# ssilverman16/particle_col_image_segmentation

Measured on AMD Instinct MI355X. Metric: Mpixels/sec segmented (5-ch 1024x1024 TIFF), ROI mask IoU=1.0, higher is better.
Workload: dtype f32 planes / u8 class maps / int32 labels / f64 ROI sums; 1 GPU; BASELINE config 2: batch of 64 frames 1024x1024x5 float32 per GPU, full kernel chain, inputs resident in HBM; frames_per_gpu=64, height=1024, width=1024, planes=5, parallelism=frames x1, launch=one hipGraph replay per step, 4 in flight, tie_fallback_frames_last_step=0, reference_nan_frames_rank0=0

## Files before the change

particle_col_image_segmentation_amd/csrc/watershed.hip:

```cpp
#include <algorithm>
#include <atomic>
#include <climits>
#include <mutex>
#include <type_traits>

#include "common.h"
#include "tile_rounds.h"

namespace pcseg {

constexpr int WS_T = 64;
constexpr unsigned WS_INF = 0xFFFFFFFFu;
constexpr int WS_CNT0 = 32, WS_CNT_STRIDE = 32, WS_CHANGED_INTS = WS_CNT0 + 16 * WS_CNT_STRIDE;

__device__ __forceinline__ unsigned ws_key(float f)
{
    if (f == 0.0f) f = 0.0f;
    unsigned u = __float_as_uint(f);
    u = (u & 0x80000000u) ? ~u : (u | 0x80000000u);
    return u == WS_INF ? WS_INF - 1 : u;
}

__global__ void __launch_bounds__(256) ws_init_kernel(const float *__restrict__ img, int64_t frame_stride,
                                                       const int *__restrict__ markers, const uint8_t *__restrict__ mask,
                                                       unsigned *__restrict__ val, unsigned *__restrict__ L,
                                                       int *__restrict__ out, int64_t n, int64_t total)
{
    int64_t i = (int64_t)blockIdx.x * blockDim.x + threadIdx.x;
    if (i >= total) return;
    bool m = mask[i] != 0;
    unsigned v = m ? ws_key(img[(i / n) * frame_stride + (i % n)]) : WS_INF;
    int mk = m ? markers[i] : 0;
    val[i] = v;
    L[i] = mk != 0 ? v : WS_INF;
    out[i] = mk;
}

constexpr int WS_LIST_SPAN = 8;
template <typename Body>
__device__ __forceinline__ void ws_for_frames(const int *frame_list, int grid_index, int grid_size, Body &&body)
{
    if (!frame_list) body(grid_index);
    else walk_list(frame_list, frame_list - 1, grid_index, grid_size, body);
}
static inline int ws_frame_span(const int *frame_list, int B) { return frame_list ? (B < WS_LIST_SPAN ? B : WS_LIST_SPAN) : B; }

constexpr int WS_TILE_GRID = 512;

template <typename Body>
__device__ __forceinline__ void ws_for_tile_pixels(int tx, int ty, int H, int W, Body &&body)
{
    const int c = tx * WS_T + (threadIdx.x & 63);
    for (int rr = threadIdx.x >> 6; rr < WS_T; rr += 4) {
        const int r = ty * WS_T + rr;
        if (r < H && c < W) body(r, c);
    }
}

struct RelaxGeom {
    static_assert(WS_T == 64, "relaxation tiles are 64 pixels wide: one wave per sweep quadrant");
    static constexpr int S = WS_T + 2;
    static constexpr int P = WS_T + 4;
    static constexpr int PAD = 8;
    static constexpr int N = S * P + 2 * PAD;
    static constexpr int THREADS = 4 * 64;
    static constexpr int HE = WS_T / 2;
    static constexpr size_t LDS_BYTES = sizeof(uint2) * N;
};

template <int DR, int DC, int P>
__device__ __forceinline__ bool ws_quadrant_sweep(uint2 *sLV, int lane)
{
    unsigned *sLw = reinterpret_cast<unsigned *>(sLV);
    typedef unsigned u2v __attribute__((ext_vector_type(2)));
    unsigned long long diff = 0;
    {
        constexpr int fr = DR > 0 ? 1 : WS_T, hr = DR > 0 ? 0 : WS_T + 1;
        const uint2 c = sLV[fr * P + 1 + lane];
        const unsigned h = sLV[hr * P + 1 + lane].x;
        const unsigned nw = min(c.x, max(c.y, h));
        atomicMin(&sLw[2 * (fr * P + 1 + lane)], nw);
        diff |= __ballot(nw != c.x);
    }
    const int lr = DR > 0 ? lane + 1 : WS_T - lane;
    const uint2 *row = sLV + lr * P;
    const unsigned halo = row[DC > 0 ? 0 : WS_T + 1].x;
    const int u0 = (0 - lane) & 63;
    unsigned left = row[DC > 0 ? u0 : WS_T + 1 - u0].x;
    const int un = (0 - (lane + 1)) & 63;
    unsigned prev = row[DC > 0 ? 1 + un : WS_T - un].x;
    const unsigned a0 = (unsigned)(uintptr_t)(row + (DC > 0 ? 1 : WS_T));
#pragma unroll 1
    for (int j0 = 0; j0 < WS_T; j0 += 8) {
        const int ub = (u0 + j0) & 63;
        const unsigned base_a = DC > 0 ? a0 + 8u * (unsigned)ub : a0 - 8u * (unsigned)ub - 56u;
        const unsigned base_b = DC > 0 ? base_a - 512u : base_a + 512u;
        unsigned ba[8];
        u2v t[8];
#define PCSEG_DS_READ(k)                                                                                                   \
        {                                                                                                                      \
            const unsigned long long wrapped = (((1ull << (k)) - 1ull) << 1) << j0;                \
            asm("v_cndmask_b32_e64 %0, %1, %2, %3" : "=v"(ba[k]) : "v"(base_a), "v"(base_b), "s"(wrapped));                     \
            asm volatile("ds_read_b64 %0, %1 offset:%2" : "=v"(t[k]) : "v"(ba[k]), "n"(DC > 0 ? 8 * (k) : 8 * (7 - (k))));     \
        }
        PCSEG_DS_READ(0) PCSEG_DS_READ(1) PCSEG_DS_READ(2) PCSEG_DS_READ(3)
        PCSEG_DS_READ(4) PCSEG_DS_READ(5) PCSEG_DS_READ(6) PCSEG_DS_READ(7)
#undef PCSEG_DS_READ
        asm volatile("s_waitcnt lgkmcnt(0)" : "+v"(t[0]), "+v"(t[1]), "+v"(t[2]), "+v"(t[3]), "+v"(t[4]), "+v"(t[5]), "+v"(t[6]), "+v"(t[7]));
        unsigned wr[8];
        unsigned long long batch_diff = 0;
#pragma unroll
        for (int k = 0; k < 8; ++k) {
            const unsigned up = (unsigned)__builtin_amdgcn_update_dpp((int)WS_INF, (int)prev, 0x138, 0xF, 0xF, false);
            const unsigned long long at0 = (1ull << k) << j0;
            unsigned lf;
            asm("v_cndmask_b32_e64 %0, %1, %2, %3" : "=v"(lf) : "v"(left), "v"(halo), "s"(at0));
            const unsigned cur = t[k].x, v = t[k].y;
            const unsigned m = min(up, lf);
            const unsigned cand = min(max(v, m), max(min(v, m), cur));
            wr[k] = cand;
            batch_diff |= __ballot(cur != cand);
            left = cand;
            prev = cand;
        }
        if (batch_diff != 0) {
#define PCSEG_DS_MIN(k)                                                                                                             \
            asm volatile("ds_min_u32 %0, %1 offset:%2" : : "v"(ba[k]), "v"(wr[k]), "n"(DC > 0 ? 8 * (k) : 8 * (7 - (k))) : "memory");
            PCSEG_DS_MIN(0) PCSEG_DS_MIN(1) PCSEG_DS_MIN(2) PCSEG_DS_MIN(3)
            PCSEG_DS_MIN(4) PCSEG_DS_MIN(5) PCSEG_DS_MIN(6) PCSEG_DS_MIN(7)
#undef PCSEG_DS_MIN
            diff |= batch_diff;
        }
    }
    return diff != 0;
}

struct WsInputs {
    const float *img;
    int64_t frame_stride;
    const int *markers;
    const uint8_t *mask;
    int *out;
    bool vec;
};


__device__ __forceinline__ void ws_relax_tile(uint2 *sLV, const WsInputs &in, const bool FIRST, unsigned *__restrict__ val,
                                              unsigned *__restrict__ L, uint8_t *__restrict__ dirty_in,
                                              uint8_t *__restrict__ dirty_out, int *__restrict__ any_changed, int H, int W,
                                              const Tiling &cur, const Tiling &nxt, int max_iter, int tx, int ty, int b,
                                              int *__restrict__ list_out = nullptr, int *__restrict__ count_out = nullptr)
{
    using G = RelaxGeom;
    constexpr int T = WS_T, S = G::S, P = G::P, NT = G::THREADS, QW = T / 4;
    const int tid = threadIdx.x;
    if (!FIRST && !take_mark(dirty_in + ((int64_t)b * cur.ny + ty) * cur.nx + tx)) return;
    if (tid == 0) atomicAdd(any_changed + WS_CNT0 + WS_CNT_STRIDE * ((tx + 5 * ty + 3 * b) & 15), 1);
    const int r0 = ty * T - cur.off, c0 = tx * T - cur.off;
    const int64_t fbase = (int64_t)b * H * W;
    auto initial = [&](int r, int c) -> uint2 {
        const int64_t g = fbase + rowoff(r, W) + c;
        if (!in.mask[g]) return make_uint2(WS_INF, WS_INF);
        const unsigned v = ws_key(in.img[(int64_t)b * in.frame_stride + rowoff(r, W) + c]);
        return make_uint2(in.markers[g] != 0 ? v : WS_INF, v);
    };
    if (in.vec) {
        constexpr int QUADS = S * QW, TRIPS = (QUADS + NT - 1) / NT;
        const float *img_f = in.img + (int64_t)b * in.frame_stride;
        const bool halo_thread = tid < 2 * S;
        const int h_lr = tid >> 1, h_lc = (tid & 1) ? S - 1 : 0;
        const int h_r = r0 + h_lr - 1, h_c = c0 + h_lc - 1;
        const bool h_in = halo_thread && h_r >= 0 && h_r < H && h_c >= 0 && h_c < W;
        const int64_t h_p = rowoff(min(max(h_r, 0), H - 1), W) + min(max(h_c, 0), W - 1);
        if (FIRST) {
            float4 f4[TRIPS];
            int4 m4[TRIPS];
            unsigned k4[TRIPS];
#pragma unroll
            for (int t = 0; t < TRIPS; ++t) {
                const int idx = min(tid + NT * t, QUADS - 1);
                const int lr = idx / QW, q = idx % QW;
                const int64_t p = rowoff(min(max(r0 + lr - 1, 0), H - 1), W) + min(max(c0 + 4 * q, 0), W - 4);
                f4[t] = *reinterpret_cast<const float4 *>(img_f + p);
                m4[t] = *reinterpret_cast<const int4 *>(in.markers + fbase + p);
                k4[t] = *reinterpret_cast<const unsigned *>(in.mask + fbase + p);
            }
            const float hf = img_f[h_p];
            const int hm = in.markers[fbase + h_p];
            const uint8_t hk = in.mask[fbase + h_p];
#pragma unroll
            for (int t = 0; t < TRIPS; ++t) {
                const int idx = tid + NT * t;
                if (idx < QUADS) {
                    const int lr = idx / QW, q = idx % QW;
                    const int r = r0 + lr - 1, c = c0 + 4 * q;
                    const bool inside = r >= 0 && r < H && c >= 0 && c < W;
                    const float fv[4] = {f4[t].x, f4[t].y, f4[t].z, f4[t].w};
                    const int mv[4] = {m4[t].x, m4[t].y, m4[t].z, m4[t].w};
                    unsigned key[4];
                    int lab[4];
#pragma unroll
                    for (int j = 0; j < 4; ++j) {
                        const bool msk = inside && ((k4[t] >> (8 * j)) & 255u) != 0;
                        key[j] = msk ? ws_key(fv[j]) : WS_INF;
                        lab[j] = msk ? mv[j] : 0;
                        sLV[lr * P + 1 + 4 * q + j] = make_uint2(lab[j] != 0 ? key[j] : WS_INF, key[j]);
                    }
                    if (inside && lr >= 1 && lr <= T) {
                        const int64_t g = fbase + rowoff(r, W) + c;
                        *reinterpret_cast<uint4 *>(val + g) = make_uint4(key[0], key[1], key[2], key[3]);
                        *reinterpret_cast<int4 *>(in.out + g) = make_int4(lab[0], lab[1], lab[2], lab[3]);
                    }
                }
            }
            if (halo_thread) {
                const bool msk = h_in && hk != 0;
                const unsigned key = msk ? ws_key(hf) : WS_INF;
                sLV[h_lr * P + h_lc] = make_uint2(msk && hm != 0 ? key : WS_INF, key);
            }
        } else {
            uint4 l4[TRIPS], v4[TRIPS];
#pragma unroll
            for (int t = 0; t < TRIPS; ++t) {
                const int idx = min(tid + NT * t, QUADS - 1);
                const int lr = idx / QW, q = idx % QW;
                const int64_t p = fbase + rowoff(min(max(r0 + lr - 1, 0), H - 1), W) + min(max(c0 + 4 * q, 0), W - 4);
                l4[t] = *reinterpret_cast<const uint4 *>(L + p);
                v4[t] = *reinterpret_cast<const uint4 *>(val + p);
            }
            const unsigned hl = L[fbase + h_p], hv = val[fbase + h_p];
#pragma unroll
            for (int t = 0; t < TRIPS; ++t) {
                const int idx = tid + NT * t;
                if (idx < QUADS) {
                    const int lr = idx / QW, q = idx % QW;
                    const int r = r0 + lr - 1, c = c0 + 4 * q;
                    const bool inside = r >= 0 && r < H && c >= 0 && c < W;
                    uint2 *dst = sLV + lr * P + 1 + 4 * q;
                    dst[0] = inside ? make_uint2(l4[t].x, v4[t].x) : make_uint2(WS_INF, WS_INF);
                    dst[1] = inside ? make_uint2(l4[t].y, v4[t].y) : make_uint2(WS_INF, WS_INF);
                    dst[2] = inside ? make_uint2(l4[t].z, v4[t].z) : make_uint2(WS_INF, WS_INF);
                    dst[3] = inside ? make_uint2(l4[t].w, v4[t].w) : make_uint2(WS_INF, WS_INF);
                }
            }
            if (halo_thread) sLV[h_lr * P + h_lc] = h_in ? make_uint2(hl, hv) : make_uint2(WS_INF, WS_INF);
        }
    } else
    for (int i = tid; i < S * S; i += NT) {
        int lr = i / S, lc = i % S;
        int r = r0 + lr - 1, c = c0 + lc - 1;
        uint2 lv = make_uint2(WS_INF, WS_INF);
        if (r >= 0 && r < H && c >= 0 && c < W) {
            if (FIRST) {
                lv = initial(r, c);
                if (lr >= 1 && lr <= T && lc >= 1 && lc <= T) {
                    const int64_t g = fbase + rowoff(r, W) + c;
                    val[g] = lv.y;
                    in.out[g] = lv.y != WS_INF ? in.markers[g] : 0;
                }
            } else {
                lv.x = L[fbase + rowoff(r, W) + c];
                lv.y = val[fbase + rowoff(r, W) + c];
            }
        }
        sLV[lr * P + lc] = lv;
    }
    __syncthreads();
    const bool rim_thread = tid < 8 * G::HE;
    const int e = tid / G::HE, ej = tid % G::HE;
    const int qy = e < 4 ? (e >> 1) : (e & 1), qx = e < 4 ? (e & 1) : ((e >> 1) & 1);
    const int rim_lr = e < 4 ? (qy ? T : 1) : qy * G::HE + ej + 1;
    const int rim_lc = e < 4 ? qx * G::HE + ej + 1 : (qx ? T : 1);
    const unsigned rim_before = rim_thread ? sLV[rim_lr * P + rim_lc].x : 0u;
    const int dir = (tid >> 6) & 3, lane = tid & 63;
    bool changed_any = false;
    bool capped = true;
    for (int iter = 0; iter < max_iter; ++iter) {
        bool changed;
        if (dir == 0) changed = ws_quadrant_sweep<1, 1, P>(sLV, lane);
        else if (dir == 1) changed = ws_quadrant_sweep<1, -1, P>(sLV, lane);
        else if (dir == 2) changed = ws_quadrant_sweep<-1, 1, P>(sLV, lane);
        else changed = ws_quadrant_sweep<-1, -1, P>(sLV, lane);
        if (!__syncthreads_or(changed)) { capped = false; break; }
        changed_any = true;
    }
    if (!FIRST && !changed_any) return;
    if (changed_any) {
        const int r = r0 + rim_lr - 1, c = c0 + rim_lc - 1;
        bool ch = rim_thread && capped;
        if (rim_thread && !capped && r >= 0 && r < H && c >= 0 && c < W) ch = sLV[rim_lr * P + rim_lc].x != rim_before;
        const unsigned long long mine = ((1ull << G::HE) - 1ull) << ((tid & 63) / G::HE * G::HE);
        const unsigned long long edge_changed = __ballot(ch) & mine;
        if (rim_thread && edge_changed && ej == 0) {
            const int oy = (r0 + qy * G::HE + nxt.off) / T, ox = (c0 + qx * G::HE + nxt.off) / T;
            if (oy >= 0 && oy < nxt.ny && ox >= 0 && ox < nxt.nx)
                mark_tile(dirty_out, list_out, count_out, ((int64_t)b * nxt.ny + oy) * nxt.nx + ox);
        }
    }
    __syncthreads();
    if (in.vec) {
#pragma unroll
        for (int t = 0; t < T * QW / NT; ++t) {
            const int idx = tid + NT * t, lr = idx / QW, q = idx % QW;
            const int r = r0 + lr, c = c0 + 4 * q;
            const uint2 *src = sLV + (lr + 1) * P + 1 + 4 * q;
            if (r >= 0 && r < H && c >= 0 && c < W)
                *reinterpret_cast<uint4 *>(L + fbase + rowoff(r, W) + c) = make_uint4(src[0].x, src[1].x, src[2].x, src[3].x);
        }
        return;
    }
    for (int i = tid; i < T * T; i += NT) {
        int lr = i / T, lc = i % T;
        int r = r0 + lr, c = c0 + lc;
        if (r >= 0 && r < H && c >= 0 && c < W) L[fbase + rowoff(r, W) + c] = sLV[(lr + 1) * P + lc + 1].x;
    }
}

__global__ void __launch_bounds__(RelaxGeom::THREADS) ws_relax_kernel(WsInputs in, const bool FIRST, unsigned *__restrict__ val,
                                                                         unsigned *__restrict__ L, uint8_t *__restrict__ dirty_in,
                                                                         uint8_t *__restrict__ dirty_out, int *__restrict__ any_changed,
                                                                         int H, int W, Tiling cur, Tiling nxt, int max_iter,
                                                                         int *__restrict__ list_out, int *__restrict__ count_out)
{
    extern __shared__ __attribute__((aligned(16))) uint2 relax_lds[];
    const TileIndex t = xcd_tile_index();
    ws_relax_tile(relax_lds + RelaxGeom::PAD, in, FIRST, val, L, dirty_in, dirty_out, any_changed, H, W, cur, nxt, max_iter, t.x, t.y,
                     t.z, list_out, count_out);
}

constexpr int WS_LIST_FROM = 4, WS_LIST_GRID = 1024;

__global__ void __launch_bounds__(RelaxGeom::THREADS) ws_relax_list_kernel(WsInputs in, unsigned *__restrict__ val, unsigned *__restrict__ L,
                                                                           uint8_t *__restrict__ dirty_in, uint8_t *__restrict__ dirty_out,
                                                                           int *__restrict__ any_changed, int H, int W, Tiling cur,
                                                                           Tiling nxt, int max_iter, TileList tiles,
                                                                           int *__restrict__ list_out, int *__restrict__ count_out)
{
    extern __shared__ __attribute__((aligned(16))) uint2 relax_lds[];
    for_tiles(tiles, [&](const int b, const int tx, const int ty) {
        ws_relax_tile(relax_lds + RelaxGeom::PAD, in, false, val, L, dirty_in, dirty_out, any_changed, H, W, cur, nxt, max_iter, tx, ty, b,
                      list_out, count_out);
        __syncthreads();
    });
}

__global__ void __launch_bounds__(RelaxGeom::THREADS) ws_relax_tail_kernel(WsInputs in, unsigned *__restrict__ val, unsigned *__restrict__ L,
                                                                           uint8_t *__restrict__ dirtyA, uint8_t *__restrict__ dirtyB,
                                                                           int *__restrict__ any_changed, int *__restrict__ not_converged,
                                                                           int *__restrict__ exact_flags, int H, int W, Tiling t0,
                                                                           Tiling t1, int first_round, int max_rounds)
{
    extern __shared__ __attribute__((aligned(16))) uint2 relax_lds[];
    const int b = blockIdx.x;
    const int rounds = tail_rounds<RelaxGeom::THREADS>(
        b, dirtyA, dirtyB, first_round, max_rounds, t0, t1, [](const int) { return true; },
        [&](const Tiling &cur, const Tiling &nxt, const int tx, const int ty, uint8_t *din, uint8_t *dout) {
            ws_relax_tile(relax_lds + RelaxGeom::PAD, in, false, val, L, din, dout, any_changed, H, W, cur, nxt, 100000, tx, ty, b);
        });
    if (rounds < 0 && threadIdx.x == 0) { *not_converged = 1; exact_flags[b] = 1; }
}

__device__ __forceinline__ bool ws_active(const uint8_t *active, int b, int r, int c, int tilesX, int tilesY)
{
    return active == nullptr || active[((int64_t)b * tilesY + r / WS_T) * tilesX + c / WS_T] != 0;
}

__global__ void __launch_bounds__(256) ws_list_tiles_kernel(const int *__restrict__ frame_list, const uint8_t *__restrict__ active, int ntpf,
                                                             int *__restrict__ tile_list)
{
    ws_for_frames(frame_list, blockIdx.x, gridDim.x, [&](const int b) {
        for (int t = threadIdx.x; t < ntpf; t += 256)
            if (active[(int64_t)b * ntpf + t]) tile_list[atomicAdd(&tile_list[-1], 1)] = b * ntpf + t;
    });
}

constexpr int UF_TW = 64, UF_TH = 32, UF_SW = UF_TW + 2, UF_SH = UF_TH + 2;
constexpr int UF_LNS = UF_TW * UF_TH;
constexpr int UF_NS = 1 << 30;

__device__ __forceinline__ int vfind_lds(int *par, int v)
{
    int p;
    while ((p = ld_lds(par + (v & (UF_LNS - 1)))) != v) {
        const int g = ld_lds(par + (p & (UF_LNS - 1)));
        if (g != p) st_lds(par + (v & (UF_LNS - 1)), g);
        v = g;
    }
    return v;
}
__device__ __forceinline__ void vunite_lds(int *par, int a, int b)
{
    for (;;) {
        a = vfind_lds(par, a);
        b = vfind_lds(par, b);
        if (a == b) return;
        if (a < b) { int t = a; a = b; b = t; }
        int old = atomicMin(&par[a & (UF_LNS - 1)], b);
        if (old == a) return;
        a = old;
    }
}
__device__ __forceinline__ bool vwalk_ok(int x, int p, int n) { return (unsigned)p <= (unsigned)x && (p & (UF_NS - 1)) < n; }

__device__ __forceinline__ void vunite_glb(int *par, int p, int q, int n, int *corrupt)
{
    int a = ld_agent(par + p), b = ld_agent(par + q);
    bool ok = a >= 0 && b >= 0 && (a & (UF_NS - 1)) < n && (b & (UF_NS - 1)) < n;
    while (ok) {
        for (;;) {
            if (a == b) return;
            const int pa = ld_agent(par + (a & (UF_NS - 1))), pb = ld_agent(par + (b & (UF_NS - 1)));
            if (pa == a && pb == b) break;
            if (!vwalk_ok(a, pa, n) || !vwalk_ok(b, pb, n)) { ok = false; break; }
            const int ga = ld_agent(par + (pa & (UF_NS - 1))), gb = ld_agent(par + (pb & (UF_NS - 1)));
            if (!vwalk_ok(pa, ga, n) || !vwalk_ok(pb, gb, n)) { ok = false; break; }
            if (pa != a) {
                if (ga != pa) __hip_atomic_store(par + (a & (UF_NS - 1)), ga, __ATOMIC_RELAXED, __HIP_MEMORY_SCOPE_AGENT);
                a = ga;
            }
            if (pb != b) {
                if (gb != pb) __hip_atomic_store(par + (b & (UF_NS - 1)), gb, __ATOMIC_RELAXED, __HIP_MEMORY_SCOPE_AGENT);
                b = gb;
            }
        }
        if (!ok) break;
        if (a == b) return;
        if (a < b) { int t = a; a = b; b = t; }
        int old = atomicMin(par + (a & (UF_NS - 1)), b);
        if (old == a) return;
        if (!vwalk_ok(a, old, n)) break;
        a = old;
    }
    walk_corrupt(corrupt);
}
__device__ __forceinline__ int vwalk_root(const int *par, int x, int n, bool &bad)
{
    int q;
    while ((q = par[x & (UF_NS - 1)]) != x) {
        if (!vwalk_ok(x, q, n)) {
            bad = true;
            break;
        }
        x = q;
    }
    return x;
}

template <typename KeyT>
__device__ __forceinline__ void ws_uf_tile_frame(KeyT *sK, int *par, uint8_t *sM, const int b, const int tile_x, const int tile_y,
                                                 const KeyT *__restrict__ K,
                                                 const int *__restrict__ F, const uint8_t *__restrict__ active,
                                                 int *__restrict__ parent, uint8_t *__restrict__ minmask, uint8_t *__restrict__ bad,
                                                 int H, int W, int tilesX, int tilesY)
{
    const KeyT KINF = ~(KeyT)0;
    const int r0 = tile_y * UF_TH, c0 = tile_x * UF_TW;
    if (!ws_active(active, b, r0, c0, tilesX, tilesY)) return;
    const int64_t fbase = (int64_t)b * H * W;
    if (sizeof(KeyT) == 4 && (W & 3) == 0 && c0 + UF_TW <= W && (((uintptr_t)K) & 15) == 0) {
        constexpr int QUADS = UF_SH * (UF_TW / 4), TRIPS = (QUADS + 255) / 256;
        uint4 kq[TRIPS];
#pragma unroll
        for (int t = 0; t < TRIPS; ++t) {
            const int i = min((int)threadIdx.x + 256 * t, QUADS - 1);
            const int r = r0 + i / (UF_TW / 4) - 1;
            kq[t] = *reinterpret_cast<const uint4 *>(K + fbase + rowoff(min(max(r, 0), H - 1), W) + c0 + 4 * (i % (UF_TW / 4)));
        }
        const int hl = min((int)threadIdx.x, UF_SH * 2 - 1);
        const int hr = r0 + (hl >> 1) - 1, hx = (hl & 1) ? UF_TW : -1, hc = c0 + hx;
        const KeyT hv = K[fbase + rowoff(min(max(hr, 0), H - 1), W) + min(max(hc, 0), W - 1)];
#pragma unroll
        for (int t = 0; t < TRIPS; ++t) {
            const int i = (int)threadIdx.x + 256 * t;
            if (i < QUADS) {
                const int lr = i / (UF_TW / 4), r = r0 + lr - 1;
                const bool in = r >= 0 && r < H;
                KeyT *dst = sK + lr * UF_SW + 1 + 4 * (i % (UF_TW / 4));
                dst[0] = in ? (KeyT)kq[t].x : KINF; dst[1] = in ? (KeyT)kq[t].y : KINF;
                dst[2] = in ? (KeyT)kq[t].z : KINF; dst[3] = in ? (KeyT)kq[t].w : KINF;
            }
        }
        if (threadIdx.x < UF_SH * 2) sK[(hl >> 1) * UF_SW + hx + 1] = (hr >= 0 && hr < H && hc >= 0 && hc < W) ? hv : KINF;
    } else {
        constexpr int TRIPS = (UF_SH * UF_SW + 255) / 256;
        KeyT kv[TRIPS];
#pragma unroll
        for (int t = 0; t < TRIPS; ++t) {
            const int i = min((int)threadIdx.x + 256 * t, UF_SH * UF_SW - 1);
            const int r = r0 + i / UF_SW - 1, c = c0 + i % UF_SW - 1;
            kv[t] = K[fbase + rowoff(min(max(r, 0), H - 1), W) + min(max(c, 0), W - 1)];
        }
#pragma unroll
        for (int t = 0; t < TRIPS; ++t) {
            const int i = (int)threadIdx.x + 256 * t;
            const int r = r0 + i / UF_SW - 1, c = c0 + i % UF_SW - 1;
            if (i < UF_SH * UF_SW) sK[i] = (r >= 0 && r < H && c >= 0 && c < W) ? kv[t] : KINF;
        }
    }
    __syncthreads();
    int self[UF_LNS / 256];
    int fv[UF_LNS / 256];
#pragma unroll
    for (int k = 0; k < UF_LNS / 256; ++k) {
        const int t = threadIdx.x + k * 256;
        fv[k] = F[fbase + rowoff(min(r0 + t / UF_TW, H - 1), W) + min(c0 + t % UF_TW, W - 1)];
    }
#pragma unroll
    for (int k = 0; k < UF_LNS / 256; ++k) {
        const int t = threadIdx.x + k * 256;
        const int lr = t / UF_TW, lc = t % UF_TW;
        const int r = r0 + lr, c = c0 + lc;
        const int i = (lr + 1) * UF_SW + lc + 1;
        int v = -1;
        if ((unsigned)(sK[i] >> (8 * sizeof(KeyT) - 32)) != WS_INF)
            v = fv[k] != 0 ? t : t + UF_LNS;
        uint8_t m8 = 0;
        if (v >= UF_LNS) {
            const KeyT ku = sK[i - UF_SW], kl = sK[i - 1], kr = sK[i + 1], kd = sK[i + UF_SW];
            const KeyT m = min(min(ku, kd), min(kl, kr));
            if (m != KINF) m8 = (ku == m ? 1 : 0) | (kl == m ? 2 : 0) | (kr == m ? 4 : 0) | (kd == m ? 8 : 0);
        }
        self[k] = v;
        sM[t] = m8;
        if (r < H && c < W) {
            minmask[fbase + rowoff(r, W) + c] = m8;
            if (fv[k] != 0) bad[fbase + rowoff(r, W) + c] = 0;
        }
    }
    __syncthreads();
#pragma unroll
    for (int k = 0; k < UF_LNS / 256; ++k) {
        const int t = threadIdx.x + k * 256;
        const int lc = t % UF_TW;
        const bool joins_left = lc > 0 && ((sM[t] & 2) || (sM[t - 1] & 4));
        const unsigned long long heads = __ballot(!joins_left);
        const unsigned long long seeds = __ballot(self[k] >= 0 && self[k] < UF_LNS);
        const unsigned long long upto = heads & (lc == 63 ? ~0ull : ((2ull << lc) - 1ull));
        const int start = 63 - __clzll((long long)upto);
        const unsigned long long later = lc == 63 ? 0ull : (heads >> (lc + 1));
        const int end = later ? lc + (__ffsll((long long)later) - 1) : 63;
        const unsigned long long run = (end == 63 ? ~0ull : ((2ull << end) - 1ull)) & ~((1ull << start) - 1ull);
        const unsigned long long run_seeds = seeds & run;
        int root = -1;
        if (self[k] >= 0) {
            if (run_seeds) root = (t - lc) + (__ffsll((long long)run_seeds) - 1);
            else root = (t - lc) + start + UF_LNS;
        }
        par[t] = root;
    }
    __syncthreads();
#pragma unroll
    for (int k = 0; k < UF_LNS / 256; ++k) {
        const int t = threadIdx.x + k * 256;
        const int lr = t / UF_TW, lc = t % UF_TW;
        if (lr == 0 || self[k] < 0) continue;
        const uint8_t m = sM[t], mu = sM[t - UF_TW];
        if (!((m & 1) || (mu & 8))) continue;
        if (lc > 0) {
            const uint8_t ml = sM[t - 1], mul = sM[t - UF_TW - 1];
            const bool same_run = (m & 2) || (ml & 4), same_run_up = (mu & 2) || (mul & 4), left_vertical = (ml & 1) || (mul & 8);
            if (same_run && same_run_up && left_vertical) continue;
        }
        vunite_lds(par, par[t], par[t - UF_TW]);
    }
    __syncthreads();
    for (int t = threadIdx.x; t < UF_TH * UF_TW; t += 256) {
        const int r = r0 + t / UF_TW, c = c0 + t % UF_TW;
        if (r >= H || c >= W) continue;
        int v = -1;
        if (par[t] >= 0) {
            const int root = vfind_lds(par, par[t]);
            const int lt = root & (UF_LNS - 1);
            v = ((r0 + lt / UF_TW) * W + c0 + lt % UF_TW) | (root >= UF_LNS ? UF_NS : 0);
        }
        parent[fbase + rowoff(r, W) + c] = v;
    }
}

template <typename KeyT, bool LIST>
__global__ void __launch_bounds__(256) ws_uf_tile_kernel(TileList tiles, const KeyT *__restrict__ K, const int *__restrict__ F,
                                                          const uint8_t *__restrict__ active, int *__restrict__ parent,
                                                          uint8_t *__restrict__ minmask, uint8_t *__restrict__ bad, int H, int W,
                                                          int tilesX, int tilesY)
{
    __shared__ KeyT sK[UF_SH * UF_SW];
    __shared__ int par[UF_TH * UF_TW];
    __shared__ uint8_t sM[UF_LNS];
// ... 1135 lines not shown
```

Before: 16780 Mpixels/s.

## Track changed rows in relaxation sweeps and confirm convergence early via row checks

Each quadrant sweep now returns a bitmask of the rows it changed instead of a single flag. On non-first visits, when only a few rows (dilated by one) changed, each wave checks those rows for any remaining fixed-point violations, and the tile stops iterating early if none are found. This is meant to save the extra full confirming sweep per tile visit. The cost is an extra barrier and the row-check work, plus the risk of stopping before true convergence if the check misses a case.

After: 17020 Mpixels/s (median of 5 runs). 1.5% higher.

```diff
diff --git a/particle_col_image_segmentation_amd/csrc/watershed.hip b/particle_col_image_segmentation_amd/csrc/watershed.hip
--- a/particle_col_image_segmentation_amd/csrc/watershed.hip
+++ b/particle_col_image_segmentation_amd/csrc/watershed.hip
@@ -69,18 +69,19 @@
 };
 
 template <int DR, int DC, int P>
-__device__ __forceinline__ bool ws_quadrant_sweep(uint2 *sLV, int lane)
+__device__ __forceinline__ unsigned long long ws_quadrant_sweep(uint2 *sLV, int lane)
 {
     unsigned *sLw = reinterpret_cast<unsigned *>(sLV);
     typedef unsigned u2v __attribute__((ext_vector_type(2)));
     unsigned long long diff = 0;
+    constexpr int fr = DR > 0 ? 1 : WS_T, hr = DR > 0 ? 0 : WS_T + 1;
+    unsigned long long first_row_diff;
     {
-        constexpr int fr = DR > 0 ? 1 : WS_T, hr = DR > 0 ? 0 : WS_T + 1;
         const uint2 c = sLV[fr * P + 1 + lane];
         const unsigned h = sLV[hr * P + 1 + lane].x;
         const unsigned nw = min(c.x, max(c.y, h));
         atomicMin(&sLw[2 * (fr * P + 1 + lane)], nw);
-        diff |= __ballot(nw != c.x);
+        first_row_diff = __ballot(nw != c.x);
     }
     const int lr = DR > 0 ? lane + 1 : WS_T - lane;
     const uint2 *row = sLV + lr * P;
@@ -132,7 +133,9 @@
             diff |= batch_diff;
         }
     }
-    return diff != 0;
+    unsigned long long rows = DR > 0 ? diff : __brevll(diff);
+    if (first_row_diff != 0) rows |= 1ull << (fr - 1);
+    return rows;
 }
 
 struct WsInputs {
@@ -144,6 +147,36 @@
     bool vec;
 };
 
+
+constexpr int WS_CONFIRM_ROWS = 16;
+
+template <int P>
+__device__ __forceinline__ bool ws_rows_violated(const uint2 *sLV, unsigned long long rows, int wave, int lane)
+{
+    unsigned long long mine = rows & (0x1111111111111111ull << __builtin_amdgcn_readfirstlane(wave));
+    const int first = __ffsll(mine);
+    bool violated = false;
+    while (mine != 0) {
+        int r[4];
+#pragma unroll
+        for (int j = 0; j < 4; ++j) {
+            const int b = __ffsll(mine);
+            mine &= mine - 1;
+            r[j] = b != 0 ? b : first;
+        }
+        uint2 c[4];
+        unsigned m[4];
+#pragma unroll
+        for (int j = 0; j < 4; ++j) {
+            const uint2 *p = sLV + r[j] * P + 1 + lane;
+            c[j] = p[0];
+            m[j] = min(min(p[-P].x, p[P].x), min(p[-1].x, p[1].x));
+        }
+#pragma unroll
+        for (int j = 0; j < 4; ++j) violated |= c[j].x > max(c[j].y, m[j]);
+    }
+    return violated;
+}
 
 __device__ __forceinline__ void ws_relax_tile(uint2 *sLV, const WsInputs &in, const bool FIRST, unsigned *__restrict__ val,
                                               unsigned *__restrict__ L, uint8_t *__restrict__ dirty_in,
@@ -275,14 +308,32 @@
     const int dir = (tid >> 6) & 3, lane = tid & 63;
     bool changed_any = false;
     bool capped = true;
+    __shared__ unsigned long long changed_rows[2][4];
+    __shared__ int row_verdict[4];
     for (int iter = 0; iter < max_iter; ++iter) {
-        bool changed;
-        if (dir == 0) changed = ws_quadrant_sweep<1, 1, P>(sLV, lane);
-        else if (dir == 1) changed = ws_quadrant_sweep<1, -1, P>(sLV, lane);
-        else if (dir == 2) changed = ws_quadrant_sweep<-1, 1, P>(sLV, lane);
-        else changed = ws_quadrant_sweep<-1, -1, P>(sLV, lane);
-        if (!__syncthreads_or(changed)) { capped = false; break; }
+        unsigned long long rows;
+        if (dir == 0) rows = ws_quadrant_sweep<1, 1, P>(sLV, lane);
+        else if (dir == 1) rows = ws_quadrant_sweep<1, -1, P>(sLV, lane);
+        else if (dir == 2) rows = ws_quadrant_sweep<-1, 1, P>(sLV, lane);
+        else rows = ws_quadrant_sweep<-1, -1, P>(sLV, lane);
+        if (lane == 0) changed_rows[iter & 1][dir] = rows;
+        __syncthreads();
+        const unsigned long long *cr = changed_rows[iter & 1];
+        const unsigned long long d = cr[0] | cr[1] | cr[2] | cr[3];
+        const unsigned long long D = (unsigned long long)(unsigned)__builtin_amdgcn_readfirstlane((unsigned)(d >> 32)) << 32 |
+                                     (unsigned)__builtin_amdgcn_readfirstlane((unsigned)d);
+        if (D == 0) { capped = false; break; }
         changed_any = true;
+        if (!FIRST) {
+            const unsigned long long suspects = D | D << 1 | D >> 1;
+            if (__popcll(suspects) <= WS_CONFIRM_ROWS) {
+                const bool wave_violated = __ballot(ws_rows_violated<P>(sLV, suspects, dir, lane)) != 0;
+                if (lane == 0) row_verdict[dir] = wave_violated;
+                __syncthreads();
+                const bool violated = __builtin_amdgcn_readfirstlane(row_verdict[0] | row_verdict[1] | row_verdict[2] | row_verdict[3]) != 0;
+                if (!violated) { capped = false; break; }
+            }
+        }
     }
     if (!FIRST && !changed_any) return;
     if (changed_any) {
diff --git a/profiles/relax_confirm/record_tie_flags.py b/profiles/relax_confirm/record_tie_flags.py
--- /dev/null
+++ b/profiles/relax_confirm/record_tie_flags.py
@@ -0,0 +1,19 @@
+import json
+import os
+import sys
+
+sys.path.insert(0, os.path.join(os.path.dirname(os.path.abspath(__file__)), "..", "..", "tests"))
+
+import test_gpu_relax_confirm as t
+from particle_col_image_segmentation_amd import ops
+
+flags = {}
+for seed in t.REGRESSION_SEEDS:
+    img, markers, mask = t.regression_inputs(ops, seed)
+    _, f = ops.watershed(img, markers, mask, mode=0)
+    flags[str(seed)] = f.cpu().tolist()
+with open(sys.argv[1], "w") as out:
+    json.dump({"library": os.environ.get("PCSEG_LIB", "this tree's"), "frames": "synth.gen_batch_torch(seed, 8, 256, 256), plane 3",
+               "tie_flags": flags}, out, indent=1)
+    out.write("\n")
+print(flags)
diff --git a/profiles/relax_confirm/row_statistics.py b/profiles/relax_confirm/row_statistics.py
--- /dev/null
+++ b/profiles/relax_confirm/row_statistics.py
@@ -0,0 +1,67 @@
+import collections
+import sys
+
+KINDS = ["round 0", "grid rounds 1-3", "list rounds", "tail"]
+WHAT = ["followed by a changing iteration", "last changing iteration of its visit", "cut at the iteration cap"]
+BINS = [str(k) for k in range(1, 17)] + ["17-24", "25-32", "33-40", "41-48", "49-56", "57-64"]
+
+
+def run():
+    import torch
+    from particle_col_image_segmentation_amd import ops, synth
+    stack = synth.gen_batch_torch(10_000, 64, 1024, 1024, torch.device("cuda", 0))
+    bm = stack[:, 3]
+    d2, mask = ops.edt_sq_lt(bm, 0.5)
+    _, markers, _ = ops.local_maxima(d2, want_mask=False)
+    torch.cuda.synchronize()
+    print("relax_row_stats_begin", flush=True)
+    labels, flags = ops.watershed(bm, markers, mask, mode=0)
+    torch.cuda.synchronize()
+    print("relax_row_stats_end labels_sum %d flags %d" % (int(labels.sum().item()), int(flags.sum().item())), flush=True)
+
+
+def read(path):
+    slots = collections.Counter()
+    for line in open(path):
+        f = line.split()
+        if len(f) == 3 and f[0] == "relax_row_stats":
+            slots[int(f[1])] += int(f[2])
+    return slots
+
+
+def table(named_logs):
+    for name, path in named_logs:
+        s = read(path)
+        print("## %s\n" % name)
+        print("| rounds | visits | tile-iterations | row tests run | row tests passed |\n|---|---|---|---|---|")
+        tot = [0, 0, 0, 0]
+        for k, kind in enumerate(KINDS):
+            v = [s[264 + 4 * k + j] for j in (3, 0, 1, 2)]
+            tot = [a + b for a, b in zip(tot, v)]
+            print("| %s | %d | %d | %d | %d |" % ((kind,) + tuple(v)))
+        print("| all | %d | %d | %d | %d |\n" % tuple(tot))
+        print("Changing iterations by the number of suspect rows (changed rows dilated by one):\n")
+        print("| rounds | what came after | " + " | ".join(BINS) + " |\n|---|---|" + "---|" * len(BINS))
+        for k, kind in enumerate(KINDS):
+            for w, what in enumerate(WHAT):
+                row = [s[66 * k + 22 * w + b] for b in range(22)]
+                if sum(row):
+                    print("| %s | %s | " % (kind, what) + " | ".join(str(x) for x in row) + " |")
+        print()
+        print("Share at or below a gate of G rows:\n")
+        print("| rounds | what came after | n | " + " | ".join("G=%d" % g for g in (4, 6, 8, 10, 12, 16, 24, 32)) + " |\n|---|---|---|" + "---|" * 8)
+        for k, kind in enumerate(KINDS):
+            for w, what in enumerate(WHAT):
+                row = [s[66 * k + 22 * w + b] for b in range(22)]
+                n = sum(row)
+                if n:
+                    cum = lambda g: sum(row[:g]) if g <= 16 else sum(row[:16 + (g - 16) // 8])
+                    print("| %s | %s | %d | " % (kind, what, n) + " | ".join("%.0f %%" % (100.0 * cum(g) / n) for g in (4, 6, 8, 10, 12, 16, 24, 32)) + " |")
+        print()
+
+
+if __name__ == "__main__":
+    if sys.argv[1:2] == ["run"]:
+        run()
+    else:
+        table([a.rsplit("=", 1) for a in sys.argv[2:]])
```
